# nateraw/pytorchvideo-accelerate

Measured on AMD Instinct MI355X. Metric: clips/sec (whole node) SlowFast-R50 32x2x224 at 1/2/4/8 MI355X; step-time p50, higher is better.
Workload: dtype bf16; 1 GPU; model=SlowFast-R50 32x2x224, global_batch=160, per_gpu_batch=160, grad_accum=1, seq_len=32, parallelism=dp1, backend=none, comm=none, forced_sync=False, grad_dtype=fp32, classes=400, hip_graph=False, deterministic=True

## Files before the change

csrc/kernels/conv_igemm.hip:

```cpp
#include "common.h"
#include "conv_params.h"
#include <type_traits>

PVA_NS_BEGIN

namespace {

__host__ __device__ constexpr int epi_rows(int BM, int BN) { return BM * BN > 128 * 128 ? 64 : BM; }

__host__ __device__ constexpr int main_lds_bytes(int BM, int BN, int BK, int EPI, int NS = 2) {
  return (EPI && epi_rows(BM, BN) * (BN * 4 + 16) > NS * (BM + BN) * BK * 2) ? epi_rows(BM, BN) * (BN * 4 + 16)
                                                                             : NS * (BM + BN) * BK * 2;
}

__host__ __device__ constexpr int dma_stages(int BM, int BN, int BK, bool dma) {
  return (dma && BM * BN == 256 * 128) ? (3 * (BM + BN) * BK * 2 <= 80 * 1024 ? 3 : 2)
         : (dma && BM * BN > 128 * 128 && 4 * (BM + BN) * BK * 2 <= 128 * 1024) ? 4
         : (dma && 3 * (BM + BN) * BK * 2 <= 96 * 1024) ? 3 : 2;
}

template <int N>
__device__ __forceinline__ void vm_wait() { asm volatile("s_waitcnt vmcnt(%0)" ::"n"(N) : "memory"); }

template <int BASE, int MAXB>
__device__ __forceinline__ void vm_wait_dyn(int nb) {
  if constexpr (MAXB <= 0) {
    vm_wait<BASE>();
  } else {
    if (nb >= MAXB) vm_wait<BASE + MAXB>();
    else vm_wait_dyn<BASE, MAXB - 1>(nb);
  }
}

__device__ __forceinline__ void dma16(__amdgpu_buffer_rsrc_t r, char* lds, int voff, int soff) {
#if defined(__HIP_DEVICE_COMPILE__)
  __builtin_amdgcn_raw_ptr_buffer_load_lds(r, (__attribute__((address_space(3))) void*)lds, 16, voff, soff, 0, 0);
#endif
}

template <int BK>
__device__ __forceinline__ int lds_swz(int row) {
  if constexpr (BK == 32) return ((row >> 2) & 1) << 1;
  else return row & 6;
}

template <int BK>
__device__ __forceinline__ int lds_off(int row, int slot) {
  if constexpr (BK == 32) return row * 64 + ((slot ^ (((row >> 2) & 1) << 1)) << 4);
  else return row * 128 + ((slot ^ (row & 6)) << 4);
}

template <int BK, int TM, int TN>
__device__ __forceinline__ void mma_ktile(const char* A, const int (&fa)[BK / 32][TM], const int (&fb)[BK / 32][TN],
                                          f32x4_t (&acc)[TM][TN]) {
  ev8_t af[2][TM], bfr[2][TN];
#pragma unroll
  for (int i = 0; i < TM; ++i) af[0][i] = *reinterpret_cast<const ev8_t*>(A + fa[0][i]);
#pragma unroll
  for (int j = 0; j < TN; ++j) bfr[0][j] = *reinterpret_cast<const ev8_t*>(A + fb[0][j]);
#pragma unroll
  for (int kk = 0; kk < BK / 32; ++kk) {
    const int c = kk & 1;
    if (kk + 1 < BK / 32) {
#pragma unroll
      for (int i = 0; i < TM; ++i) af[c ^ 1][i] = *reinterpret_cast<const ev8_t*>(A + fa[kk + 1][i]);
#pragma unroll
      for (int j = 0; j < TN; ++j) bfr[c ^ 1][j] = *reinterpret_cast<const ev8_t*>(A + fb[kk + 1][j]);
      __builtin_amdgcn_sched_barrier(0);
    }
#pragma unroll
    for (int i = 0; i < TM; ++i)
#pragma unroll
      for (int j = 0; j < TN; ++j)
        acc[i][j] = PVA_MFMA16(bfr[c][j], af[c][i], acc[i][j], 0, 0, 0);
  }
}

template <int BM, int BN, int WM, int WN, int CH, int BK, int EPI, int UT>
__global__ __launch_bounds__((BM / WM) * (BN / WN) * 64, (BM * BN == 256 * 128) ? 2 : 1)
void conv_igemm_kernel(const ConvParams p) {
  constexpr int NWN = BN / WN;
  constexpr int NT = (BM / WM) * NWN * 64;
  constexpr int CPR = BK / CH;
  constexpr int A_CHUNKS = BM * CPR, B_CHUNKS = BN * CPR;
  constexpr int A_SLOTS = (A_CHUNKS + NT - 1) / NT;
  constexpr int B_SLOTS = (B_CHUNKS + NT - 1) / NT;
  constexpr int TM = WM / 16, TN = WN / 16;
  constexpr int TILE_BYTES = (BM + BN) * BK * 2;
  constexpr int STG_PITCH = BN * 4 + 16;
  constexpr int NSTAGE = dma_stages(BM, BN, BK, (UT & 17) == 17);
  constexpr int MAIN_BYTES = main_lds_bytes(BM, BN, BK, EPI, NSTAGE);
  static_assert(NT % CPR == 0, "thread count must be a multiple of chunks per row");
  using VT = typename std::conditional<CH == 8, uint4, uint2>::type;

  extern __shared__ __attribute__((aligned(16))) char smem[];
  constexpr int NWAVES = (BM / WM) * NWN;
  constexpr int RED_FLOATS = EPI >= 1 ? NWAVES * 3 * BN : (BM / WM) * 2 * BN;
  float* red = reinterpret_cast<float*>(smem + MAIN_BYTES);
  float* bnp = red + RED_FLOATS;
  float* aff = bnp + (EPI >= 1 ? 6 * BN : 0);

  const int tid = threadIdx.x, lane = tid & 63, wid = tid >> 6;
  const int wm = wid / NWN, wn = wid % NWN;
  const int n_tiles = (p.Ngemm + BN - 1) / BN;
  const int nwg = gridDim.x;
  const int t = xcd_remap(blockIdx.x, nwg);
  const int tile_m = t / n_tiles, tile_n = t % n_tiles;
  const int m0 = tile_m * BM, n0 = tile_n * BN;

  const bool do_stats = EPI == 0 && p.stats != nullptr;
  const bool do_bstats = EPI >= 1 && p.epart != nullptr;
  const int affine = p.affine;
  if (do_bstats) {
    for (int i = tid; i < BN; i += NT) {
      const int n = n0 + i;
      const bool ok = n < p.Ngemm, d = ok && p.ey1 != nullptr, d0 = ok && p.ey0 != nullptr;
      bnp[i] = d0 ? p.emean0[n] : 0.f;
      bnp[BN + i] = d0 ? p.erstd0[n] : 0.f;
      bnp[2 * BN + i] = d ? p.emean1[n] : 0.f;
      bnp[3 * BN + i] = d ? p.erstd1[n] : 0.f;
      bnp[4 * BN + i] = (ok && p.emsc) ? p.emsc[n] : 0.f;
      bnp[5 * BN + i] = (ok && p.emsh) ? p.emsh[n] : 0.f;
    }
  }
  if (affine) {
    for (int i = tid; i < p.Cg; i += NT) { aff[i] = p.in_scale[i]; aff[p.Cg + i] = p.in_shift[i]; }
  }

  const int RHW = p.Rh * p.Rw, RTHW = p.Rt * RHW;
  f32x4_t acc[TM][TN];
#pragma unroll
  for (int i = 0; i < TM; ++i)
#pragma unroll
    for (int j = 0; j < TN; ++j) acc[i][j] = f32x4_t{0.f, 0.f, 0.f, 0.f};
  const int frow = lane & 15, fslot = lane >> 4;
  int fa[BK / 32][TM], fb[BK / 32][TN];
#pragma unroll
  for (int kk = 0; kk < BK / 32; ++kk) {
#pragma unroll
    for (int i = 0; i < TM; ++i) fa[kk][i] = lds_off<BK>(wm * WM + i * 16 + frow, fslot + 4 * kk);
#pragma unroll
    for (int j = 0; j < TN; ++j) fb[kk][j] = BM * BK * 2 + lds_off<BK>(wn * WN + j * 16 + frow, fslot + 4 * kk);
  }

  if constexpr (UT & 1) {
    static_assert(CH == 8, "uniform-tap loader stages 16-B chunks");
    const __amdgpu_buffer_rsrc_t xr = __builtin_amdgcn_make_buffer_rsrc((void*)p.x, (short)0, (int)p.xbytes, 0x00020000);
    const __amdgpu_buffer_rsrc_t wr = __builtin_amdgcn_make_buffer_rsrc((void*)p.w, (short)0, (int)p.wbytes, 0x00020000);
    constexpr unsigned OOB = 0xFFFFFFF0u;
    const int col = tid % CPR;
    constexpr bool check = (UT >> 1) & 1;
    constexpr int uaff = (UT >> 2) & 3;
    constexpr bool glds_ut = (UT >> 4) & 1;
    static_assert(!glds_ut || uaff == 0, "LDS-DMA staging cannot transform the A operand");
    const int GHW = p.Gh * p.Gw, GTHW = p.Gt * GHW;
    const int tmin = p.dir < 0 ? -(((p.nt - 1) * p.Gh + (p.nh - 1)) * p.Gw + (p.nw - 1)) * p.ldx : 0;
    int a_vo[A_SLOTS], sa[A_SLOTS];
    unsigned tmask[A_SLOTS];
#pragma unroll
    for (int s = 0; s < A_SLOTS; ++s) {
      const int idx = tid + s * NT;
      const int row = idx / CPR;
      const int m = m0 + row;
      const bool rv = idx < A_CHUNKS && m < p.M;
      int at = 0, ah = 0, aw = 0, off = 0;
      if (rv) {
        const int b = pva_fdiv(m, p.mg_thw, p.sh_thw);
        int r = m - b * RTHW;
        const int qt = pva_fdiv(r, p.mg_hw, p.sh_hw); r -= qt * RHW;
        const int qh = pva_fdiv(r, p.mg_w, p.sh_w); const int qw = r - qh * p.Rw;
        at = qt * p.ast + p.aot; ah = qh * p.ash + p.aoh; aw = qw * p.asw + p.aow;
        off = (b * GTHW + (at * p.Gh + ah) * p.Gw + aw) * p.ldx + (glds_ut ? col ^ lds_swz<BK>(row) : col) * 8;
      }
      unsigned msk = 0;
      if (check && rv) {
        int t = 0;
        for (int jt = 0; jt < p.nt; ++jt)
          for (int jh = 0; jh < p.nh; ++jh)
            for (int jw = 0; jw < p.nw; ++jw, ++t)
              if ((unsigned)(at + p.dir * jt) < (unsigned)p.Gt && (unsigned)(ah + p.dir * jh) < (unsigned)p.Gh &&
                  (unsigned)(aw + p.dir * jw) < (unsigned)p.Gw)
                msk |= 1u << t;
      }
      tmask[s] = msk;
// ... 317 lines not shown
      a_off[s] = 0; a_t[s] = 0; a_h[s] = 0; a_w[s] = 0;
      if (idx < A_CHUNKS && m < p.M) {
        const int b = pva_fdiv(m, p.mg_thw, p.sh_thw);
        int r = m - b * RTHW;
        const int qt = pva_fdiv(r, p.mg_hw, p.sh_hw); r -= qt * RHW;
        const int qh = pva_fdiv(r, p.mg_w, p.sh_w); const int qw = r - qh * p.Rw;
        a_t[s] = qt * p.ast + p.aot; a_h[s] = qh * p.ash + p.aoh; a_w[s] = qw * p.asw + p.aow;
        a_off[s] = (b * GTHW + (a_t[s] * p.Gh + a_h[s]) * p.Gw + a_w[s]) * p.ldx;
        rowok |= 1u << s;
      }
      if constexpr (CH == 8) sa[s] = lds_off<BK>(row, col);
      else sa[s] = lds_off<BK>(row, col >> 1) + (col & 1) * 8;
    }
    int b_off[B_SLOTS], sb[B_SLOTS];
    unsigned nok = 0;
  #pragma unroll
    for (int s = 0; s < B_SLOTS; ++s) {
      const int idx = tid + s * NT;
      const int row = idx / CPR;
      const int n = n0 + row;
      b_off[s] = n * p.Kfull;
      if (idx < B_CHUNKS && n < p.Ngemm) nok |= 1u << s;
      if constexpr (CH == 8) sb[s] = lds_off<BK>(row, col);
      else sb[s] = lds_off<BK>(row, col >> 1) + (col & 1) * 8;
    }
  
    int kc = col * CH, kdt = 0, kdh = 0, kdw = 0;
    int tap_lin = 0, tap_w = 0;
    auto retap = [&]() {
      tap_lin = p.dir * ((kdt * p.Gh + kdh) * p.Gw + kdw) * p.ldx;
      tap_w = (((p.bt0 + kdt * p.bts) * p.kh + (p.bh0 + kdh * p.bhs)) * p.kw + (p.bw0 + kdw * p.bws)) * p.Cg;
    };
    auto kadvance = [&](int by) {
      kc += by;
      if (kc >= p.Cg) {
        do {
          kc -= p.Cg;
          if (++kdw == p.nw) { kdw = 0; if (++kdh == p.nh) { kdh = 0; ++kdt; } }
        } while (kc >= p.Cg);
        retap();
      }
    };
    retap();
    kadvance(0);
  
    VT ra[A_SLOTS], rb[B_SLOTS];
    int ra_c = 0;
    unsigned ra_valid = 0;
  
    auto load = [&]() {
      const bool tap_ok = kdt < p.nt;
      ra_c = kc; ra_valid = 0;
      const int dgt = p.dir * kdt, dgh = p.dir * kdh, dgw = p.dir * kdw;
  #pragma unroll
      for (int s = 0; s < A_SLOTS; ++s) {
        bool v = tap_ok & ((rowok >> s & 1) != 0);
        if (check)
          v = v & ((unsigned)(a_t[s] + dgt) < (unsigned)p.Gt) & ((unsigned)(a_h[s] + dgh) < (unsigned)p.Gh) &
              ((unsigned)(a_w[s] + dgw) < (unsigned)p.Gw);
        ra[s] = *reinterpret_cast<const VT*>(p.x + (v ? a_off[s] + tap_lin + kc : 0));
        ra_valid |= (unsigned)v << s;
      }
      const int boff = tap_w + kc;
  #pragma unroll
      for (int s = 0; s < B_SLOTS; ++s) {
        if (tap_ok && (nok >> s & 1))
          rb[s] = *reinterpret_cast<const VT*>(p.w + (b_off[s] + boff));
        else
          rb[s] = VT{};
      }
      kadvance(BK);
    };
  
    auto store_lds = [&](int buf) {
      char* A = smem + buf * TILE_BYTES;
      char* B = A + BM * BK * 2;
      float asc[CH], ash[CH];
      if (affine) {
  #pragma unroll
        for (int e = 0; e < CH; ++e) { asc[e] = aff[ra_c + e]; ash[e] = aff[p.Cg + ra_c + e]; }
      }
      const uint32_t rfloor = affine == 2 ? 0u : 0x80008000u;
  #pragma unroll
      for (int s = 0; s < A_SLOTS; ++s) {
        if constexpr (A_CHUNKS % NT != 0) if (tid + s * NT >= A_CHUNKS) break;
        VT v = ra[s];
        const uint32_t keep = 0u - ((ra_valid >> s) & 1u);
        if (!affine) {
          if constexpr (CH == 8) v = make_uint4(v.x & keep, v.y & keep, v.z & keep, v.w & keep);
          else v = make_uint2(v.x & keep, v.y & keep);
        } else {
          float f[CH];
          if constexpr (CH == 8) unpack8(v, f); else unpack4(v, f);
  #pragma unroll
          for (int e = 0; e < CH; ++e) f[e] = __builtin_fmaf(f[e], asc[e], ash[e]);
          if constexpr (CH == 8) {
            v = pack8_fast(f);
            v = make_uint4(max_e16x2(v.x, rfloor) & keep, max_e16x2(v.y, rfloor) & keep,
                           max_e16x2(v.z, rfloor) & keep, max_e16x2(v.w, rfloor) & keep);
          } else {
            v = make_uint2(max_e16x2(cvt_pk_e16(f[0], f[1]), rfloor) & keep,
                           max_e16x2(cvt_pk_e16(f[2], f[3]), rfloor) & keep);
          }
        }
        *reinterpret_cast<VT*>(A + sa[s]) = v;
      }
  #pragma unroll
      for (int s = 0; s < B_SLOTS; ++s) {
        if constexpr (B_CHUNKS % NT != 0) if (tid + s * NT >= B_CHUNKS) break;
        *reinterpret_cast<VT*>(B + sb[s]) = rb[s];
      }
    };
  
  
    const int nsteps = (p.nt * p.nh * p.nw * p.Cg + BK - 1) / BK;
    __syncthreads();
    load();
    store_lds(0);
    if (nsteps > 1) load();

    for (int step = 0; step < nsteps; ++step) {
      const int cur = step & 1;
      __syncthreads();
      if (step + 1 < nsteps) {
        store_lds(cur ^ 1);
        if (step + 2 < nsteps) load();
      }
      const char* A = smem + cur * TILE_BYTES;
  #pragma unroll
      for (int kk = 0; kk < BK / 32; ++kk) {
        ev8_t af[TM], bfr[TN];
  #pragma unroll
        for (int i = 0; i < TM; ++i) af[i] = *reinterpret_cast<const ev8_t*>(A + fa[kk][i]);
  #pragma unroll
        for (int j = 0; j < TN; ++j) bfr[j] = *reinterpret_cast<const ev8_t*>(A + fb[kk][j]);
  #pragma unroll
        for (int i = 0; i < TM; ++i)
  #pragma unroll
          for (int j = 0; j < TN; ++j)
            acc[i][j] = PVA_MFMA16(bfr[j], af[i], acc[i][j], 0, 0, 0);
      }
    }
  }
  if constexpr ((UT >> 5) & 3) vm_wait<0>();
  if constexpr (EPI >= 1) __syncthreads();

  float cs[TN][4], cq[TN][4];
#pragma unroll
  for (int j = 0; j < TN; ++j)
#pragma unroll
    for (int r = 0; r < 4; ++r) { cs[j][r] = 0.f; cq[j][r] = 0.f; }

  const bool dense_rows = p.ost == 1 && p.osh == 1 && p.osw == 1 && p.Rt == p.Ot && p.Rh == p.Oh && p.Rw == p.Ow;
#pragma unroll
  for (int i = 0; i < TM; ++i) {
    const int m = m0 + wm * WM + i * 16 + frow;
    int pos = m;
    if (!dense_rows && m < p.M) {
      const int b = pva_fdiv(m, p.mg_thw, p.sh_thw);
      int r = m - b * RTHW;
      const int qt = pva_fdiv(r, p.mg_hw, p.sh_hw); r -= qt * RHW;
      const int qh = pva_fdiv(r, p.mg_w, p.sh_w); const int qw = r - qh * p.Rw;
      pos = ((b * p.Ot + qt * p.ost + p.ort) * p.Oh + qh * p.osh + p.orh) * p.Ow + qw * p.osw + p.orw;
    }
    if constexpr (EPI == 0) {
#pragma unroll
      for (int j = 0; j < TN; ++j) {
        const int n = n0 + wn * WN + j * 16 + 4 * fslot;
        float v[4] = {acc[i][j][0], acc[i][j][1], acc[i][j][2], acc[i][j][3]};
        if (p.fres) {
          const bool ok = m < p.M && n < p.Ngemm;
          unsigned bits = 0;
          if (ok) {
            const f32x4_t sc = *reinterpret_cast<const f32x4_t*>(p.fsc + n);
            const f32x4_t sh = *reinterpret_cast<const f32x4_t*>(p.fsh + n);
            float r[4];
            unpack4(*reinterpret_cast<const uint2*>(p.eres + pos * p.ldr + n), r);
            if (p.rsc) {
              const f32x4_t rs = *reinterpret_cast<const f32x4_t*>(p.rsc + n);
              const f32x4_t rh = *reinterpret_cast<const f32x4_t*>(p.rsh + n);
#pragma unroll
              for (int e = 0; e < 4; ++e) r[e] = r[e] * rs[e] + rh[e];
            }
#pragma unroll
            for (int e = 0; e < 4; ++e) v[e] = fmaxf(v[e] * sc[e] + sh[e] + r[e], 0.f);
            const uint2 pk = pack4(v);
            *reinterpret_cast<uint2*>(p.y + pos * p.ldy + n) = pk;
            const uint32_t w2[2] = {pk.x, pk.y};
#pragma unroll
            for (int e = 0; e < 2; ++e) {
              bits |= ((w2[e] & 0x7fffu) != 0 && !(w2[e] & 0x8000u)) ? 1u << (2 * e) : 0u;
              bits |= ((w2[e] & 0x7fff0000u) != 0 && !(w2[e] & 0x80000000u)) ? 1u << (2 * e + 1) : 0u;
            }
          }
          const unsigned other = swap_partner16(bits);
          if (ok && !(fslot & 1)) p.emask_out[pos * (p.Ngemm >> 3) + (n >> 3)] = (uint8_t)(bits | (other << 4));
          continue;
        }
        if (m < p.M && n < p.Ngemm) {
          uint16_t* dst = p.y + pos * p.ldy + n;
          if (p.ebias) {
            const f32x4_t b = *reinterpret_cast<const f32x4_t*>(p.ebias + n);
#pragma unroll
            for (int r = 0; r < 4; ++r) v[r] += b[r];
          }
          if (p.accum) {
            float o[4];
            unpack4(*reinterpret_cast<const uint2*>(dst), o);
#pragma unroll
            for (int r = 0; r < 4; ++r) v[r] += o[r];
          }
          const uint2 pk = pack4(v);
          if (!p.nostore) *reinterpret_cast<uint2*>(dst) = pk;
          if (do_stats) {
            float q[4];
            unpack4(pk, q);
#pragma unroll
            for (int r = 0; r < 4; ++r) { cs[j][r] += q[r]; cq[j][r] += q[r] * q[r]; }
          }
        }
      }
    }
  }
  if constexpr (EPI >= 1) {
    constexpr int CPRW = BN / 8, RPP = NT / CPRW;
    constexpr int SR = epi_rows(BM, BN);
    static_assert(NT % CPRW == 0, "rows per pass");
    static_assert(SR % 16 == 0 && SR % RPP == 0, "staging slices hold whole fragments and row passes");
    const int cg = tid % CPRW, r0 = tid / CPRW;
    const int n = n0 + cg * 8;
    float sv[8], s0[8], s1[8];
#pragma unroll
    for (int e = 0; e < 8; ++e) { sv[e] = 0.f; s0[e] = 0.f; s1[e] = 0.f; }
    const bool nok = n < p.Ngemm;
    const bool dual = EPI == 1 && p.ey1 != nullptr;
    const bool masky = EPI == 1 && do_bstats && p.emsc != nullptr;
    constexpr int RB = (EPI == 2 || BM * BN <= 128 * 128) ? 4 : 2;
#pragma unroll
    for (int r_lo = 0; r_lo < BM; r_lo += SR) {
    if (r_lo > 0) __syncthreads();
#pragma unroll
    for (int i = 0; i < TM; ++i) {
      const int row = wm * WM + i * 16 + frow;
      if (row < r_lo || row >= r_lo + SR) continue;
#pragma unroll
      for (int j = 0; j < TN; ++j) {
        const int col = wn * WN + j * 16 + 4 * fslot;
        *reinterpret_cast<f32x4_t*>(smem + (row - r_lo) * STG_PITCH + col * 4) = acc[i][j];
      }
    }
    __syncthreads();
    for (int base = r_lo + r0; base < r_lo + SR && nok; base += RB * RPP) {
      uint4 lo[RB], lr[RB], l0[RB], l1[RB];
      unsigned bits[RB];
      int pos[RB];
      bool ok[RB];
#pragma unroll
      for (int u = 0; u < RB; ++u) {
        const int rr = base + u * RPP;
        const int m = m0 + rr;
        ok[u] = rr < r_lo + SR && m < p.M;
        int ps = m;
        if (!dense_rows && ok[u]) {
          const int b = pva_fdiv(m, p.mg_thw, p.sh_thw);
          int r = m - b * RTHW;
          const int qt = pva_fdiv(r, p.mg_hw, p.sh_hw); r -= qt * RHW;
          const int qh = pva_fdiv(r, p.mg_w, p.sh_w); const int qw = r - qh * p.Rw;
          ps = ((b * p.Ot + qt * p.ost + p.ort) * p.Oh + qh * p.osh + p.orh) * p.Ow + qw * p.osw + p.orw;
        }
        pos[u] = ps;
        lo[u] = lr[u] = l0[u] = l1[u] = uint4{0, 0, 0, 0};
        bits[u] = 0xffu;
        if (ok[u]) {
          if (EPI == 1 && p.accum) lo[u] = *reinterpret_cast<const uint4*>(p.y + ps * p.ldy + n);
          if (p.eres) lr[u] = *reinterpret_cast<const uint4*>(p.eres + ps * p.ldr + n);
          if (p.emask) bits[u] = p.emask[ps * (p.Ngemm >> 3) + (n >> 3)];
          if (EPI == 1 && do_bstats) {
            if (p.ey0) l0[u] = *reinterpret_cast<const uint4*>(p.ey0 + ps * p.Ngemm + n);
            if (dual) l1[u] = *reinterpret_cast<const uint4*>(p.ey1 + ps * p.Ngemm + n);
          }
        }
      }
#pragma unroll
      for (int u = 0; u < RB; ++u) {
        if (!ok[u]) continue;
        const int rr = base + u * RPP - r_lo;
        const f32x4_t va = *reinterpret_cast<const f32x4_t*>(smem + rr * STG_PITCH + cg * 32);
        const f32x4_t vb = *reinterpret_cast<const f32x4_t*>(smem + rr * STG_PITCH + cg * 32 + 16);
        float v[8] = {va[0], va[1], va[2], va[3], vb[0], vb[1], vb[2], vb[3]};
        float o[8], rs[8];
        unpack8(lo[u], o);
        unpack8(lr[u], rs);
        if (masky) {
          float a[8];
          unpack8(l0[u], a);
#pragma unroll
          for (int e = 0; e < 8; ++e)
            if (!(a[e] * bnp[4 * BN + cg * 8 + e] + bnp[5 * BN + cg * 8 + e] > 0.f)) bits[u] &= ~(1u << e);
        }
        if (EPI == 1 && p.ebias) {
          const f32x4_t b0 = *reinterpret_cast<const f32x4_t*>(p.ebias + n);
          const f32x4_t b1 = *reinterpret_cast<const f32x4_t*>(p.ebias + n + 4);
#pragma unroll
          for (int e = 0; e < 4; ++e) { rs[e] += b0[e]; rs[e + 4] += b1[e]; }
        }
#pragma unroll
        for (int e = 0; e < 8; ++e) {
          const float t = v[e] + o[e] + rs[e];
          v[e] = (bits[u] >> e) & 1u ? t : 0.f;
        }
        const uint4 pk = pack8(v);
        *reinterpret_cast<uint4*>(p.y + pos[u] * p.ldy + n) = pk;
        if (do_bstats) {
          float q[8], a[8];
          unpack8(pk, q);
          unpack8(l0[u], a);
#pragma unroll
          for (int e = 0; e < 8; ++e) { sv[e] += q[e]; s0[e] += q[e] * a[e]; }
          if (dual) {
            unpack8(l1[u], a);
#pragma unroll
            for (int e = 0; e < 8; ++e) s1[e] += q[e] * a[e];
          }
        }
      }
    }
    }
    if (do_bstats && nok) {
#pragma unroll
      for (int e = 0; e < 8; ++e) {
        const int c = cg * 8 + e;
        s0[e] = (s0[e] - bnp[c] * sv[e]) * bnp[BN + c];
        s1[e] = (s1[e] - bnp[2 * BN + c] * sv[e]) * bnp[3 * BN + c];
      }
    }
    if (do_bstats) {
      static_assert(CPRW <= 64 && (CPRW & (CPRW - 1)) == 0, "channel groups per row");
#pragma unroll
      for (int e = 0; e < 8; ++e) {
        sv[e] = wave_sum_stride(sv[e], CPRW);
        s0[e] = wave_sum_stride(s0[e], CPRW);
        s1[e] = wave_sum_stride(s1[e], CPRW);
      }
      if (lane < CPRW) {
        float* slot = red + wid * 3 * BN;
#pragma unroll
        for (int e = 0; e < 8; ++e) {
          slot[cg * 8 + e] = sv[e];
          slot[BN + cg * 8 + e] = s0[e];
          slot[2 * BN + cg * 8 + e] = s1[e];
        }
      }
      __syncthreads();
      for (int i = tid; i < BN; i += NT) {
        const int nn = n0 + i;
        if (nn < p.Ngemm) {
#pragma unroll
          for (int k = 0; k < 3; ++k) {
            float t = 0.f;
#pragma unroll
            for (int w = 0; w < NWAVES; ++w) t += red[(w * 3 + k) * BN + i];
            p.epart[(tile_m * 3 + k) * p.Ngemm + nn] = t;
          }
        }
      }
    }
    return;
  }
  if (do_stats) {
#pragma unroll
    for (int j = 0; j < TN; ++j)
#pragma unroll
      for (int r = 0; r < 4; ++r) {
        const float s = sum16(cs[j][r]);
        const float q = sum16(cq[j][r]);
        if (frow == 0) {
          const int nl = wn * WN + j * 16 + 4 * fslot + r;
          red[wm * 2 * BN + nl] = s;
          red[wm * 2 * BN + BN + nl] = q;
        }
      }
    asm volatile("s_waitcnt lgkmcnt(0)" ::: "memory");
    __builtin_amdgcn_s_barrier();
    asm volatile("" ::: "memory");
    for (int i = tid; i < BN; i += NT) {
      const int n = n0 + i;
      if (n < p.Ngemm) {
        float s = 0.f, q = 0.f;
#pragma unroll
        for (int w = 0; w < BM / WM; ++w) { s += red[w * 2 * BN + i]; q += red[w * 2 * BN + BN + i]; }
        p.stats[(tile_m * 2) * p.Ngemm + n] = s;
        p.stats[(tile_m * 2 + 1) * p.Ngemm + n] = q;
      }
    }
  }
}

#ifndef PVA_KERNEL_ONLY
static int g_ut_mode = 1;

inline bool conv_ut_legal(const ConvParams& p, int ch, int bk) {
  return ch == 8 && p.Cg % bk == 0 && p.nt * p.nh * p.nw <= 32;
}

template <int BM, int BN, int WM, int WN, int CH, int BK>
void launch_cfg(const ConvParams& p, int ut_force, hipStream_t stream, bool dma = false, bool pf = false) {
  constexpr int NT = (BM / WM) * (BN / WN) * 64;
  const int m_tiles = (p.M + BM - 1) / BM, n_tiles = (p.Ngemm + BN - 1) / BN;
  const bool epi = !p.fres && (p.eres || p.emask || p.epart);
  constexpr int NW = (BM / WM) * (BN / WN);
  const size_t red_bytes = epi ? (NW * 3 + 6) * BN * 4 : (BM / WM) * 2 * BN * 4;
  const bool use_dma = CH == 8 && dma && !p.affine && conv_ut_legal(p, CH, BK) && ut_force != 0;
  constexpr bool PF_OK = BM * BN >= 256 * 128 && BK == 64 && CH == 8;
  const bool use_pf = PF_OK && pf && use_dma;
  const size_t lds = main_lds_bytes(BM, BN, BK, epi ? 1 : 0, dma_stages(BM, BN, BK, use_dma)) + red_bytes +
                     (p.affine ? 2 * p.Cg * 4 : 0) + (use_pf ? NW * 256 : 0);
  const dim3 grid(m_tiles * n_tiles), block(NT);
  const bool ut_legal = conv_ut_legal(p, CH, BK);
  const bool ut_pays = !p.check || (p.nt == 1 && p.ash == 1 && p.asw == 1);
  const bool ut = ut_legal && (ut_force >= 0 ? ut_force == 1 : (g_ut_mode == 2 || (g_ut_mode == 1 && ut_pays)));
  constexpr bool BIG = BM * BN > 128 * 128;
  if constexpr (BIG) {
    if (epi) {
      const bool lean = !p.accum && !p.ey0 && !p.ey1 && !p.emsc && !p.ebias;
      if (lean && ut) {
        if (dma && use_pf) {
          if constexpr (PF_OK) {
            if (p.check) hipLaunchKernelGGL((conv_igemm_kernel<BM, BN, WM, WN, CH, BK, 2, 115>), grid, block, lds, stream, p);
            else hipLaunchKernelGGL((conv_igemm_kernel<BM, BN, WM, WN, CH, BK, 2, 113>), grid, block, lds, stream, p);
          }
        } else if (dma) {
          if (p.check) hipLaunchKernelGGL((conv_igemm_kernel<BM, BN, WM, WN, CH, BK, 2, 19>), grid, block, lds, stream, p);
          else hipLaunchKernelGGL((conv_igemm_kernel<BM, BN, WM, WN, CH, BK, 2, 17>), grid, block, lds, stream, p);
        } else {
          if (p.check) hipLaunchKernelGGL((conv_igemm_kernel<BM, BN, WM, WN, CH, BK, 2, 3>), grid, block, lds, stream, p);
          else hipLaunchKernelGGL((conv_igemm_kernel<BM, BN, WM, WN, CH, BK, 2, 1>), grid, block, lds, stream, p);
        }
        return;
      }
      if (ut && dma && use_pf) {
        if constexpr (PF_OK) {
          if (p.check) hipLaunchKernelGGL((conv_igemm_kernel<BM, BN, WM, WN, CH, BK, 1, 115>), grid, block, lds, stream, p);
          else hipLaunchKernelGGL((conv_igemm_kernel<BM, BN, WM, WN, CH, BK, 1, 113>), grid, block, lds, stream, p);
        }
      } else if (ut && dma) {
        if (p.check) hipLaunchKernelGGL((conv_igemm_kernel<BM, BN, WM, WN, CH, BK, 1, 19>), grid, block, lds, stream, p);
        else hipLaunchKernelGGL((conv_igemm_kernel<BM, BN, WM, WN, CH, BK, 1, 17>), grid, block, lds, stream, p);
      } else if (ut && p.check) {
        hipLaunchKernelGGL((conv_igemm_kernel<BM, BN, WM, WN, CH, BK, 1, 3>), grid, block, lds, stream, p);
      } else if (ut) {
        hipLaunchKernelGGL((conv_igemm_kernel<BM, BN, WM, WN, CH, BK, 1, 1>), grid, block, lds, stream, p);
      } else {
        hipLaunchKernelGGL((conv_igemm_kernel<BM, BN, WM, WN, CH, BK, 1, 0>), grid, block, lds, stream, p);
      }
      return;
    }
    if (ut && dma && !p.affine && use_pf) {
      if constexpr (PF_OK) {
        if (p.check) hipLaunchKernelGGL((conv_igemm_kernel<BM, BN, WM, WN, CH, BK, 0, 115>), grid, block, lds, stream, p);
        else hipLaunchKernelGGL((conv_igemm_kernel<BM, BN, WM, WN, CH, BK, 0, 113>), grid, block, lds, stream, p);
      }
    } else if (ut && dma && !p.affine) {
      if (p.check) hipLaunchKernelGGL((conv_igemm_kernel<BM, BN, WM, WN, CH, BK, 0, 19>), grid, block, lds, stream, p);
      else hipLaunchKernelGGL((conv_igemm_kernel<BM, BN, WM, WN, CH, BK, 0, 17>), grid, block, lds, stream, p);
    } else if (ut) {
      switch ((p.check ? 2 : 0) | (p.affine << 2)) {
        case 0: hipLaunchKernelGGL((conv_igemm_kernel<BM, BN, WM, WN, CH, BK, 0, 1>), grid, block, lds, stream, p); break;
        case 2: hipLaunchKernelGGL((conv_igemm_kernel<BM, BN, WM, WN, CH, BK, 0, 3>), grid, block, lds, stream, p); break;
        case 4: hipLaunchKernelGGL((conv_igemm_kernel<BM, BN, WM, WN, CH, BK, 0, 5>), grid, block, lds, stream, p); break;
        case 6: hipLaunchKernelGGL((conv_igemm_kernel<BM, BN, WM, WN, CH, BK, 0, 7>), grid, block, lds, stream, p); break;
        case 8: hipLaunchKernelGGL((conv_igemm_kernel<BM, BN, WM, WN, CH, BK, 0, 9>), grid, block, lds, stream, p); break;
        default: hipLaunchKernelGGL((conv_igemm_kernel<BM, BN, WM, WN, CH, BK, 0, 11>), grid, block, lds, stream, p); break;
      }
    } else {
      hipLaunchKernelGGL((conv_igemm_kernel<BM, BN, WM, WN, CH, BK, 0, 0>), grid, block, lds, stream, p);
    }
    return;
  } else if constexpr (CH == 8) {
    if (ut && dma && !p.affine) {
      if (epi) {
        if (p.check) hipLaunchKernelGGL((conv_igemm_kernel<BM, BN, WM, WN, CH, BK, 1, 19>), grid, block, lds, stream, p);
        else hipLaunchKernelGGL((conv_igemm_kernel<BM, BN, WM, WN, CH, BK, 1, 17>), grid, block, lds, stream, p);
      } else {
        if (p.check) hipLaunchKernelGGL((conv_igemm_kernel<BM, BN, WM, WN, CH, BK, 0, 19>), grid, block, lds, stream, p);
        else hipLaunchKernelGGL((conv_igemm_kernel<BM, BN, WM, WN, CH, BK, 0, 17>), grid, block, lds, stream, p);
      }
      return;
    }
    if (epi) {
      if (ut && p.check) hipLaunchKernelGGL((conv_igemm_kernel<BM, BN, WM, WN, CH, BK, 1, 3>), grid, block, lds, stream, p);
      else if (ut) hipLaunchKernelGGL((conv_igemm_kernel<BM, BN, WM, WN, CH, BK, 1, 1>), grid, block, lds, stream, p);
      else hipLaunchKernelGGL((conv_igemm_kernel<BM, BN, WM, WN, CH, BK, 1, 0>), grid, block, lds, stream, p);
    } else if (ut) {
      switch ((p.check ? 2 : 0) | (p.affine << 2)) {
        case 0: hipLaunchKernelGGL((conv_igemm_kernel<BM, BN, WM, WN, CH, BK, 0, 1>), grid, block, lds, stream, p); break;
        case 2: hipLaunchKernelGGL((conv_igemm_kernel<BM, BN, WM, WN, CH, BK, 0, 3>), grid, block, lds, stream, p); break;
        case 4: hipLaunchKernelGGL((conv_igemm_kernel<BM, BN, WM, WN, CH, BK, 0, 5>), grid, block, lds, stream, p); break;
        case 6: hipLaunchKernelGGL((conv_igemm_kernel<BM, BN, WM, WN, CH, BK, 0, 7>), grid, block, lds, stream, p); break;
        case 8: hipLaunchKernelGGL((conv_igemm_kernel<BM, BN, WM, WN, CH, BK, 0, 9>), grid, block, lds, stream, p); break;
        default: hipLaunchKernelGGL((conv_igemm_kernel<BM, BN, WM, WN, CH, BK, 0, 11>), grid, block, lds, stream, p); break;
      }
    } else {
      hipLaunchKernelGGL((conv_igemm_kernel<BM, BN, WM, WN, CH, BK, 0, 0>), grid, block, lds, stream, p);
    }
  } else {
    hipLaunchKernelGGL((conv_igemm_kernel<BM, BN, WM, WN, CH, BK, 0, 0>), grid, block, lds, stream, p);
  }
}

template <int CH, int BK>
void launch_variant(int v, const ConvParams& p, int ut_force, hipStream_t stream, bool dma = false, bool pf = false) {
  switch (v) {
    case 0: launch_cfg<128, 128, 64, 64, CH, BK>(p, ut_force, stream, dma); break;
    case 1: launch_cfg<128, 64, 64, 32, CH, BK>(p, ut_force, stream, dma); break;
    case 2: launch_cfg<256, 32, 64, 32, CH, BK>(p, ut_force, stream, dma); break;
    case 4:
      if constexpr (CH == 8) launch_cfg<256, 256, 128, 64, CH, BK>(p, ut_force, stream, dma, pf);
      break;
    case 5:
      if constexpr (CH == 8) launch_cfg<256, 128, 128, 64, CH, BK>(p, ut_force, stream, dma, pf);
      break;
    default: launch_cfg<256, 16, 64, 16, CH, BK>(p, ut_force, stream, dma); break;
  }
}

#endif
}

#ifndef PVA_KERNEL_ONLY
static int pick_variant(int M, int N) {
  if (N > 64) return 0;
  if (N > 32) return 1;
  if (N > 16) return 2;
  return 3;
}

int conv_direct_rows(int cfg);
// ... 72 lines not shown
```

Measured before the change: 1288 clips/s.

## Prefetch conv epilogue loads via buffer ops with OOB masking and software pipelining

```diff
diff --git a/csrc/kernels/conv_igemm.hip b/csrc/kernels/conv_igemm.hip
--- a/csrc/kernels/conv_igemm.hip
+++ b/csrc/kernels/conv_igemm.hip
@@ -30,6 +30,40 @@
     if (nb >= MAXB) vm_wait<BASE + MAXB>();
     else vm_wait_dyn<BASE, MAXB - 1>(nb);
   }
+}
+
+constexpr unsigned EPI_OOB = 0xFFFFFFF0u;
+__device__ __forceinline__ __amdgpu_buffer_rsrc_t epi_rsrc(const void* ptr) {
+  return __builtin_amdgcn_make_buffer_rsrc(const_cast<void*>(ptr), (short)0, ptr ? (int)EPI_OOB : 0, 0x00020000);
+}
+__device__ __forceinline__ uint4 epi_ld16(__amdgpu_buffer_rsrc_t r, unsigned off) {
+  return __builtin_bit_cast(uint4, __builtin_amdgcn_raw_buffer_load_b128(r, (int)off, 0, 0));
+}
+__device__ __forceinline__ uint2 epi_ld8(__amdgpu_buffer_rsrc_t r, unsigned off) {
+  return __builtin_bit_cast(uint2, __builtin_amdgcn_raw_buffer_load_b64(r, (int)off, 0, 0));
+}
+__device__ __forceinline__ void epi_st16(__amdgpu_buffer_rsrc_t r, unsigned off, const uint4& v) {
+  __builtin_amdgcn_raw_buffer_store_b128(__builtin_bit_cast(decltype(__builtin_amdgcn_raw_buffer_load_b128(r, 0, 0, 0)), v),
+                                         r, (int)off, 0, 0);
+}
+__device__ __forceinline__ void epi_st8(__amdgpu_buffer_rsrc_t r, unsigned off, const uint2& v) {
+  __builtin_amdgcn_raw_buffer_store_b64(__builtin_bit_cast(decltype(__builtin_amdgcn_raw_buffer_load_b64(r, 0, 0, 0)), v),
+                                        r, (int)off, 0, 0);
+}
+
+__device__ __forceinline__ unsigned epi_oob(bool ok) { return ok ? 0u : EPI_OOB; }
+
+template <int ROWS, int RPS>
+__host__ __device__ constexpr int epi_upto(int k, int epi, bool big) {
+  const int sl = k / RPS;
+  const int ahead = !big ? 4 : (epi == 2 ? 3 + 4 * sl : (sl < 3 ? 1 : 3));
+  return k + ahead < ROWS - 1 ? k + ahead : ROWS - 1;
+}
+
+__device__ __forceinline__ void lds_barrier() {
+  asm volatile("s_waitcnt lgkmcnt(0)" ::: "memory");
+  __builtin_amdgcn_s_barrier();
+  asm volatile("" ::: "memory");
 }
 
 __device__ __forceinline__ void dma16(__amdgpu_buffer_rsrc_t r, char* lds, int voff, int soff) {
@@ -653,74 +687,151 @@
     for (int r = 0; r < 4; ++r) { cs[j][r] = 0.f; cq[j][r] = 0.f; }
 
   const bool dense_rows = p.ost == 1 && p.osh == 1 && p.osw == 1 && p.Rt == p.Ot && p.Rh == p.Oh && p.Rw == p.Ow;
-#pragma unroll
-  for (int i = 0; i < TM; ++i) {
-    const int m = m0 + wm * WM + i * 16 + frow;
-    int pos = m;
-    if (!dense_rows && m < p.M) {
-      const int b = pva_fdiv(m, p.mg_thw, p.sh_thw);
-      int r = m - b * RTHW;
-      const int qt = pva_fdiv(r, p.mg_hw, p.sh_hw); r -= qt * RHW;
-      const int qh = pva_fdiv(r, p.mg_w, p.sh_w); const int qw = r - qh * p.Rw;
-      pos = ((b * p.Ot + qt * p.ost + p.ort) * p.Oh + qh * p.osh + p.orh) * p.Ow + qw * p.osw + p.orw;
-    }
-    if constexpr (EPI == 0) {
-#pragma unroll
-      for (int j = 0; j < TN; ++j) {
-        const int n = n0 + wn * WN + j * 16 + 4 * fslot;
-        float v[4] = {acc[i][j][0], acc[i][j][1], acc[i][j][2], acc[i][j][3]};
-        if (p.fres) {
-          const bool ok = m < p.M && n < p.Ngemm;
+  auto out_row = [&](int row, int& pos) -> bool {
+    const int m = m0 + row;
+    const bool ok = m < p.M;
+    const int mc = ok ? m : 0;
+    const int b = pva_fdiv(mc, p.mg_thw, p.sh_thw);
+    int r = mc - b * RTHW;
+    const int qt = pva_fdiv(r, p.mg_hw, p.sh_hw); r -= qt * RHW;
+    const int qh = pva_fdiv(r, p.mg_w, p.sh_w); const int qw = r - qh * p.Rw;
+    const int sp = ((b * p.Ot + qt * p.ost + p.ort) * p.Oh + qh * p.osh + p.orh) * p.Ow + qw * p.osw + p.orw;
+    pos = dense_rows ? m : sp;
+    return ok;
+  };
+  if constexpr (EPI == 0) {
+    const __amdgpu_buffer_rsrc_t yr = epi_rsrc(p.y);
+    int ncol[TN];
+    bool nokc[TN];
+    unsigned colm[TN];
+#pragma unroll
+    for (int j = 0; j < TN; ++j) {
+      ncol[j] = n0 + wn * WN + j * 16 + 4 * fslot;
+      nokc[j] = ncol[j] < p.Ngemm;
+      colm[j] = epi_oob(nokc[j]);
+    }
+    auto frag = [&](int i, int j, float (&v)[4]) {
+      f32x4_t a = acc[i][j];
+      asm volatile("" : "+v"(a));
+      v[0] = a[0]; v[1] = a[1]; v[2] = a[2]; v[3] = a[3];
+    };
+    constexpr int NF = TM * TN;
+    constexpr int AHW = TN > 2 ? 4 : 2;
+    constexpr int AH = NF - 1 < AHW ? NF - 1 : AHW;
+    if (p.fres) {
+      const __amdgpu_buffer_rsrc_t rr = epi_rsrc(p.eres), mr = epi_rsrc(p.emask_out);
+      const int mld = p.Ngemm >> 3;
+      int pos[TM];
+      unsigned rokm = 0;
+#pragma unroll
+      for (int i = 0; i < TM; ++i) rokm |= out_row(wm * WM + i * 16 + frow, pos[i]) ? 1u << i : 0u;
+      auto frag_off = [&](int i, int j, int ld) -> unsigned {
+        return ((unsigned)(pos[i] * ld + ncol[j]) * 2u) | epi_oob((rokm >> i) & 1u) | colm[j];
+      };
+      {
+        const bool raff = p.rsc != nullptr;
+        const float* rscp = raff ? p.rsc : p.fsc;
+        const float* rshp = raff ? p.rsh : p.fsh;
+        constexpr bool CPF = TN > 2;
+        f32x4_t cst[2][4];
+        auto consts = [&](int j) {
+          const int nc = nokc[j] ? ncol[j] : 0;
+          const int c = CPF ? j & 1 : 0;
+          cst[c][0] = *reinterpret_cast<const f32x4_t*>(p.fsc + nc);
+          cst[c][1] = *reinterpret_cast<const f32x4_t*>(p.fsh + nc);
+          cst[c][2] = *reinterpret_cast<const f32x4_t*>(rscp + nc);
+          cst[c][3] = *reinterpret_cast<const f32x4_t*>(rshp + nc);
+        };
+        uint2 res[NF];
+        auto issue = [&](int q) { res[q] = epi_ld8(rr, frag_off(q % TM, q / TM, p.ldr)); };
+        consts(0);
+#pragma unroll
+        for (int q = 0; q < AH; ++q) issue(q);
+#pragma unroll
+        for (int q = 0; q < NF; ++q) {
+          const int j = q / TM, i = q % TM;
+          if (q + AH < NF) issue(q + AH);
+          if (i == 0 && (CPF ? j + 1 < TN : j > 0)) consts(CPF ? j + 1 : j);
+          const int c = CPF ? j & 1 : 0;
+          const bool ok = ((rokm >> i) & 1u) && nokc[j];
+          float v[4];
+          frag(i, j, v);
+          float r[4];
+          unpack4(res[q], r);
+          if (raff) {
+#pragma unroll
+            for (int e = 0; e < 4; ++e) r[e] = r[e] * cst[c][2][e] + cst[c][3][e];
+          }
+#pragma unroll
+          for (int e = 0; e < 4; ++e) v[e] = fmaxf(v[e] * cst[c][0][e] + cst[c][1][e] + r[e], 0.f);
+          const uint2 pk = pack4(v);
+          epi_st8(yr, frag_off(i, j, p.ldy), pk);
+          const uint32_t w2[2] = {pk.x, pk.y};
           unsigned bits = 0;
-          if (ok) {
-            const f32x4_t sc = *reinterpret_cast<const f32x4_t*>(p.fsc + n);
-            const f32x4_t sh = *reinterpret_cast<const f32x4_t*>(p.fsh + n);
-            float r[4];
-            unpack4(*reinterpret_cast<const uint2*>(p.eres + pos * p.ldr + n), r);
-            if (p.rsc) {
-              const f32x4_t rs = *reinterpret_cast<const f32x4_t*>(p.rsc + n);
-              const f32x4_t rh = *reinterpret_cast<const f32x4_t*>(p.rsh + n);
-#pragma unroll
-              for (int e = 0; e < 4; ++e) r[e] = r[e] * rs[e] + rh[e];
-            }
-#pragma unroll
-            for (int e = 0; e < 4; ++e) v[e] = fmaxf(v[e] * sc[e] + sh[e] + r[e], 0.f);
-            const uint2 pk = pack4(v);
-            *reinterpret_cast<uint2*>(p.y + pos * p.ldy + n) = pk;
-            const uint32_t w2[2] = {pk.x, pk.y};
-#pragma unroll
-            for (int e = 0; e < 2; ++e) {
-              bits |= ((w2[e] & 0x7fffu) != 0 && !(w2[e] & 0x8000u)) ? 1u << (2 * e) : 0u;
-              bits |= ((w2[e] & 0x7fff0000u) != 0 && !(w2[e] & 0x80000000u)) ? 1u << (2 * e + 1) : 0u;
-            }
+#pragma unroll
+          for (int e = 0; e < 2; ++e) {
+            bits |= ((w2[e] & 0x7fffu) != 0 && !(w2[e] & 0x8000u)) ? 1u << (2 * e) : 0u;
+            bits |= ((w2[e] & 0x7fff0000u) != 0 && !(w2[e] & 0x80000000u)) ? 1u << (2 * e + 1) : 0u;
           }
+          bits = ok ? bits : 0u;
           const unsigned other = swap_partner16(bits);
-          if (ok && !(fslot & 1)) p.emask_out[pos * (p.Ngemm >> 3) + (n >> 3)] = (uint8_t)(bits | (other << 4));
-          continue;
-        }
-        if (m < p.M && n < p.Ngemm) {
-          uint16_t* dst = p.y + pos * p.ldy + n;
-          if (p.ebias) {
-            const f32x4_t b = *reinterpret_cast<const f32x4_t*>(p.ebias + n);
-#pragma unroll
-            for (int r = 0; r < 4; ++r) v[r] += b[r];
+          __builtin_amdgcn_raw_buffer_store_b8((uint8_t)(bits | (other << 4)), mr,
+                                               (int)((unsigned)(pos[i] * mld + (ncol[j] >> 3)) | epi_oob(ok && !(fslot & 1))), 0, 0);
+        }
+      }
+    } else {
+      const bool hasb = p.ebias != nullptr;
+      auto run = [&](auto ACC) {
+        constexpr bool ACCUM = decltype(ACC)::value;
+        f32x4_t bias[TN];
+        if (hasb) {
+#pragma unroll
+          for (int j = 0; j < TN; ++j) bias[j] = *reinterpret_cast<const f32x4_t*>(p.ebias + (nokc[j] ? ncol[j] : 0));
+        }
+        int pos[TM];
+        bool rok[TM];
+        auto frag_off = [&](int i, int j) -> unsigned {
+          return ((unsigned)(pos[i] * p.ldy + ncol[j]) * 2u) | epi_oob(rok[i]) | colm[j];
+        };
+        uint2 old[NF];
+        constexpr int LEAD = ACCUM ? AH : 0;
+        auto reach = [&](int f) {
+          if (f % TN == 0) rok[f / TN] = out_row(wm * WM + (f / TN) * 16 + frow, pos[f / TN]);
+          if constexpr (ACCUM) old[f] = epi_ld8(yr, frag_off(f / TN, f % TN));
+        };
+#pragma unroll
+        for (int f = 0; f < LEAD; ++f) reach(f);
+#pragma unroll
+        for (int q = 0; q < NF; ++q) {
+          const int i = q / TN, j = q % TN;
+          if (q + LEAD < NF) reach(q + LEAD);
+          float v[4];
+          frag(i, j, v);
+          if (hasb) {
+#pragma unroll
+            for (int r = 0; r < 4; ++r) v[r] += bias[j][r];
           }
-          if (p.accum) {
+          if constexpr (ACCUM) {
             float o[4];
-            unpack4(*reinterpret_cast<const uint2*>(dst), o);
+            unpack4(old[q], o);
 #pragma unroll
             for (int r = 0; r < 4; ++r) v[r] += o[r];
           }
           const uint2 pk = pack4(v);
-          if (!p.nostore) *reinterpret_cast<uint2*>(dst) = pk;
+          const unsigned yo = frag_off(i, j);
+          epi_st8(yr, p.nostore ? EPI_OOB : yo, pk);
           if (do_stats) {
-            float q[4];
-            unpack4(pk, q);
-#pragma unroll
-            for (int r = 0; r < 4; ++r) { cs[j][r] += q[r]; cq[j][r] += q[r] * q[r]; }
+            float t[4];
+            unpack4(pk, t);
+#pragma unroll
+            for (int r = 0; r < 4; ++r) {
+              const float tt = yo < EPI_OOB ? t[r] : 0.f;
+              cs[j][r] += tt; cq[j][r] += tt * tt;
+            }
           }
         }
-      }
+      };
+      if (p.accum) run(std::true_type{}); else run(std::false_type{});
     }
   }
   if constexpr (EPI >= 1) {
@@ -736,10 +847,42 @@
     const bool nok = n < p.Ngemm;
     const bool dual = EPI == 1 && p.ey1 != nullptr;
     const bool masky = EPI == 1 && do_bstats && p.emsc != nullptr;
-    constexpr int RB = (EPI == 2 || BM * BN <= 128 * 128) ? 4 : 2;
-#pragma unroll
-    for (int r_lo = 0; r_lo < BM; r_lo += SR) {
-    if (r_lo > 0) __syncthreads();
+    const bool hasmask = p.emask != nullptr;
+    constexpr int ROWS = BM / RPP, RPS = SR / RPP;
+    static_assert(RPS >= 1 && ROWS % RPS == 0, "whole row passes per slice");
+    const __amdgpu_buffer_rsrc_t yr = epi_rsrc(p.y), oldr = epi_rsrc(EPI == 1 && p.accum ? p.y : nullptr),
+                                 rsr = epi_rsrc(p.eres), mkr = epi_rsrc(p.emask),
+                                 y0r = epi_rsrc(EPI == 1 && do_bstats ? p.ey0 : nullptr),
+                                 y1r = epi_rsrc(dual && do_bstats ? p.ey1 : nullptr);
+    f32x4_t eb0 = {0.f, 0.f, 0.f, 0.f}, eb1 = {0.f, 0.f, 0.f, 0.f};
+    if (EPI == 1 && p.ebias) {
+      eb0 = *reinterpret_cast<const f32x4_t*>(p.ebias + (nok ? n : 0));
+      eb1 = *reinterpret_cast<const f32x4_t*>(p.ebias + (nok ? n : 0) + 4);
+    }
+    uint4 lo[ROWS], lr[ROWS], l0[ROWS], l1[ROWS];
+    unsigned lbits[ROWS], yo[ROWS];
+    auto issue = [&](int k) {
+      int ps;
+      const bool ok = out_row(r0 + k * RPP, ps) && nok;
+      const unsigned oob = epi_oob(ok);
+      yo[k] = ((unsigned)(ps * p.ldy + n) * 2u) | oob;
+      lo[k] = l0[k] = l1[k] = uint4{0, 0, 0, 0};
+      if constexpr (EPI == 1) lo[k] = epi_ld16(oldr, yo[k]);
+      lr[k] = epi_ld16(rsr, ((unsigned)(ps * p.ldr + n) * 2u) | oob);
+      lbits[k] = __builtin_amdgcn_raw_buffer_load_b8(mkr, (int)((unsigned)(ps * (p.Ngemm >> 3) + (n >> 3)) | oob), 0, 0);
+      if constexpr (EPI == 1) {
+        const unsigned o01 = ((unsigned)(ps * p.Ngemm + n) * 2u) | oob;
+        l0[k] = epi_ld16(y0r, o01);
+        l1[k] = epi_ld16(y1r, o01);
+      }
+    };
+#pragma unroll
+    for (int k = 0; k < ROWS; ++k)
+      if (k <= epi_upto<ROWS, RPS>(0, EPI, BM * BN > 128 * 128)) issue(k);
+#pragma unroll
+    for (int sl = 0; sl < BM / SR; ++sl) {
+    const int r_lo = sl * SR;
+    if (sl > 0) lds_barrier();
 #pragma unroll
     for (int i = 0; i < TM; ++i) {
       const int row = wm * WM + i * 16 + frow;
@@ -750,81 +893,54 @@
         *reinterpret_cast<f32x4_t*>(smem + (row - r_lo) * STG_PITCH + col * 4) = acc[i][j];
       }
     }
-    __syncthreads();
-    for (int base = r_lo + r0; base < r_lo + SR && nok; base += RB * RPP) {
-      uint4 lo[RB], lr[RB], l0[RB], l1[RB];
-      unsigned bits[RB];
-      int pos[RB];
-      bool ok[RB];
-#pragma unroll
-      for (int u = 0; u < RB; ++u) {
-        const int rr = base + u * RPP;
-        const int m = m0 + rr;
-        ok[u] = rr < r_lo + SR && m < p.M;
-        int ps = m;
-        if (!dense_rows && ok[u]) {
-          const int b = pva_fdiv(m, p.mg_thw, p.sh_thw);
-          int r = m - b * RTHW;
-          const int qt = pva_fdiv(r, p.mg_hw, p.sh_hw); r -= qt * RHW;
-          const int qh = pva_fdiv(r, p.mg_w, p.sh_w); const int qw = r - qh * p.Rw;
-          ps = ((b * p.Ot + qt * p.ost + p.ort) * p.Oh + qh * p.osh + p.orh) * p.Ow + qw * p.osw + p.orw;
-        }
-        pos[u] = ps;
-        lo[u] = lr[u] = l0[u] = l1[u] = uint4{0, 0, 0, 0};
-        bits[u] = 0xffu;
-        if (ok[u]) {
-          if (EPI == 1 && p.accum) lo[u] = *reinterpret_cast<const uint4*>(p.y + ps * p.ldy + n);
-          if (p.eres) lr[u] = *reinterpret_cast<const uint4*>(p.eres + ps * p.ldr + n);
-          if (p.emask) bits[u] = p.emask[ps * (p.Ngemm >> 3) + (n >> 3)];
-          if (EPI == 1 && do_bstats) {
-            if (p.ey0) l0[u] = *reinterpret_cast<const uint4*>(p.ey0 + ps * p.Ngemm + n);
-            if (dual) l1[u] = *reinterpret_cast<const uint4*>(p.ey1 + ps * p.Ngemm + n);
-          }
-        }
-      }
-#pragma unroll
-      for (int u = 0; u < RB; ++u) {
-        if (!ok[u]) continue;
-        const int rr = base + u * RPP - r_lo;
+    lds_barrier();
+#pragma unroll
+    for (int u = 0; u < RPS; ++u) {
+        const int k = sl * RPS + u;
+        if (k > 0) {
+#pragma unroll
+          for (int q = 0; q < ROWS; ++q)
+            if (q > epi_upto<ROWS, RPS>(k - 1, EPI, BM * BN > 128 * 128) &&
+                q <= epi_upto<ROWS, RPS>(k, EPI, BM * BN > 128 * 128)) issue(q);
+        }
+        const int rr = r0 + u * RPP;
         const f32x4_t va = *reinterpret_cast<const f32x4_t*>(smem + rr * STG_PITCH + cg * 32);
         const f32x4_t vb = *reinterpret_cast<const f32x4_t*>(smem + rr * STG_PITCH + cg * 32 + 16);
         float v[8] = {va[0], va[1], va[2], va[3], vb[0], vb[1], vb[2], vb[3]};
         float o[8], rs[8];
-        unpack8(lo[u], o);
-        unpack8(lr[u], rs);
+        unpack8(lo[k], o);
+        unpack8(lr[k], rs);
+        unsigned bits = yo[k] < EPI_OOB ? (hasmask ? lbits[k] : 0xffu) : 0u;
         if (masky) {
           float a[8];
-          unpack8(l0[u], a);
+          unpack8(l0[k], a);
 #pragma unroll
           for (int e = 0; e < 8; ++e)
-            if (!(a[e] * bnp[4 * BN + cg * 8 + e] + bnp[5 * BN + cg * 8 + e] > 0.f)) bits[u] &= ~(1u << e);
+            if (!(a[e] * bnp[4 * BN + cg * 8 + e] + bnp[5 * BN + cg * 8 + e] > 0.f)) bits &= ~(1u << e);
         }
         if (EPI == 1 && p.ebias) {
-          const f32x4_t b0 = *reinterpret_cast<const f32x4_t*>(p.ebias + n);
-          const f32x4_t b1 = *reinterpret_cast<const f32x4_t*>(p.ebias + n + 4);
-#pragma unroll
-          for (int e = 0; e < 4; ++e) { rs[e] += b0[e]; rs[e + 4] += b1[e]; }
+#pragma unroll
+          for (int e = 0; e < 4; ++e) { rs[e] += eb0[e]; rs[e + 4] += eb1[e]; }
         }
 #pragma unroll
         for (int e = 0; e < 8; ++e) {
           const float t = v[e] + o[e] + rs[e];
-          v[e] = (bits[u] >> e) & 1u ? t : 0.f;
+          v[e] = (bits >> e) & 1u ? t : 0.f;
         }
         const uint4 pk = pack8(v);
-        *reinterpret_cast<uint4*>(p.y + pos[u] * p.ldy + n) = pk;
+        epi_st16(yr, yo[k], pk);
         if (do_bstats) {
           float q[8], a[8];
           unpack8(pk, q);
-          unpack8(l0[u], a);
+          unpack8(l0[k], a);
 #pragma unroll
           for (int e = 0; e < 8; ++e) { sv[e] += q[e]; s0[e] += q[e] * a[e]; }
           if (dual) {
-            unpack8(l1[u], a);
+            unpack8(l1[k], a);
 #pragma unroll
             for (int e = 0; e < 8; ++e) s1[e] += q[e] * a[e];
           }
         }
-      }
     }
     }
     if (do_bstats && nok) {
@@ -852,7 +968,7 @@
           slot[2 * BN + cg * 8 + e] = s1[e];
         }
       }
-      __syncthreads();
+      lds_barrier();
       for (int i = tid; i < BN; i += NT) {
         const int nn = n0 + i;
         if (nn < p.Ngemm) {
@@ -881,9 +997,7 @@
           red[wm * 2 * BN + BN + nl] = q;
         }
       }
-    asm volatile("s_waitcnt lgkmcnt(0)" ::: "memory");
-    __builtin_amdgcn_s_barrier();
-    asm volatile("" ::: "memory");
+    lds_barrier();
     for (int i = tid; i < BN; i += NT) {
       const int n = n0 + i;
       if (n < p.Ngemm) {
```

Result: no change. 1300 clips/s, median of 6 (+1.0%).
